# lab-emi/CleanUMamba

Hardware: AMD Instinct MI355X
Metric: audio samples/sec/node (train step, E8, 10s@16kHz) (higher is better)
Workload: dtype f16; 1 GPU; CleanUMamba-E8 (41.4M) full train step: fwd + L1 + multi-res STFT loss + bwd + grad all-reduce + clip + Adam; 10 s @ 16 kHz clips; global_batch=16, batch_per_gpu=16, clip_samples=160000, parallelism=dp1, weights=random init (reference init, seed 0)

## Files before the change

cleanumamba_amd/csrc/gemm_tn.hip:

```cpp
#include "common.h"

namespace cum {

typedef __attribute__((ext_vector_type(8))) __bf16 bf16x8;
typedef __attribute__((ext_vector_type(4))) __bf16 bf16x4;
typedef __attribute__((ext_vector_type(8))) _Float16 f16x8;
typedef __attribute__((ext_vector_type(4))) _Float16 f16x4;
typedef __attribute__((ext_vector_type(4))) float f32x4;

struct TnParams {
  const void *dZ, *X;
  float *slab;
  float *bslab;
  int64_t ldz, ldx;
  int64_t M;
  int N, K;
  int Np, Kp;
  int rows_per_split, nsplit;
#ifdef CUM_AB
  int skip_store;
#endif
};

constexpr int TN_T = 128;

template <typename T>
struct TnCfg;
template <>
struct TnCfg<__bf16> {
  static constexpr int EPC = 8, BMK = 64;
  static __device__ __forceinline__ int swz(int row) { return 2 * ((row & 3) | (((row >> 3) & 1) << 2)); }
};
template <>
struct TnCfg<f16> : TnCfg<__bf16> {};
template <>
struct TnCfg<float> {
  static constexpr int EPC = 4, BMK = 32;
  static __device__ __forceinline__ int swz(int row) { return 4 * (row & 7); }
};

template <typename T>
__global__ __launch_bounds__(256) __attribute__((amdgpu_waves_per_eu(sizeof(T) == 4 ? 2 : 3, 3))) void gemm_tn_kernel(const TnParams p) {
  constexpr int EPC = TnCfg<T>::EPC, BMK = TnCfg<T>::BMK;
  constexpr int CPR = TN_T / EPC;
// ... 579 lines not shown
#undef CUM_MFMA
#undef CUM_HALFQ
#undef CUM_BIAS
#undef CUM_STAGE

  float *slab = p.slab + (int64_t)sp * p.Np * p.Kp;
#pragma unroll
  for (int ni = 0; ni < 4; ++ni) {
    const int n = n0 + wn * 64 + ni * 16 + r;
#pragma unroll
    for (int h = 0; h < 2; ++h)
#pragma unroll
      for (int ki = 0; ki < 4; ++ki) {
        const int k = k0 + wk * 128 + h * 64 + ki * 16 + 4 * g;
        *reinterpret_cast<float4 *>(slab + (int64_t)n * p.Kp + k) =
            make_float4(acc[h][ni][ki][0], acc[h][ni][ki][1], acc[h][ni][ki][2], acc[h][ni][ki][3]);
      }
  }
  if (bias_wave) p.bslab[(int64_t)sp * p.Np + n0 + wn * 64 + 16 * g + r] = bacc[0];
}

#endif

template <typename T>
__global__ __launch_bounds__(512) void gemm_tn9_kernel(const TnParams p) {
  static_assert(sizeof(T) == 2, "16-bit element types only");
  constexpr int UNIT = 64 * 16;
  __shared__ uint4 lds_all[2 * 4 * UNIT];

  const int tid = threadIdx.x, lane = tid & 63;
  const int wave = uniform(tid >> 6);
  const int wk = wave >> 2, wn = wave & 3;
  const int g = lane >> 4, r = lane & 15;
  const int ntn = p.Np / 256, ntk = p.Kp / 256, tiles = ntn * ntk;
  const int w = (int)(blockIdx.x & 7) * (int)(gridDim.x >> 3) + (int)(blockIdx.x >> 3);
  if (w >= tiles * p.nsplit) return;
  const int sp = w / tiles, tile = w % tiles;
  const int n0 = (tile % ntn) * 256, k0 = (tile / ntn) * 256;
  const int64_t m_begin = (int64_t)sp * p.rows_per_split;
  int64_t m_end = m_begin + p.rows_per_split;
  m_end = m_end < p.M ? m_end : p.M;
  const int len = (int)(m_end - m_begin);
  const int nk = (len + 63) / 64;
  const int rem = len - 64 * (nk - 1);
  const T *dZ = static_cast<const T *>(p.dZ);
  const T *X = static_cast<const T *>(p.X);
  const bool bias_wave = p.bslab != nullptr && k0 == 0 && wk == 0;

  typedef __attribute__((address_space(3))) void *lds_ptr;
  typedef const __attribute__((address_space(1))) void *glb_ptr;
  const int64_t stepx = 128 * p.ldx, stepz = 128 * p.ldz;
  const char *xb = reinterpret_cast<const char *>(X + k0) + m_begin * p.ldx * 2;
  const char *zb = reinterpret_cast<const char *>(dZ + n0) + m_begin * p.ldz * 2;
  unsigned xo[2], zo[2];
#pragma unroll
  for (int it = 0; it < 2; ++it) {
    const int pos = it * 512 + tid;
    const int row = pos >> 4;
    const int clog = (pos & 15) ^ TnCfg<T>::swz(row);
    const int rowc = row < rem ? row : rem - 1;
// ... 193 lines not shown
#endif
  float *slab = p.slab + (int64_t)sp * p.Np * p.Kp;
#pragma unroll
  for (int ni = 0; ni < 4; ++ni) {
    const int n = n0 + wn * 64 + ni * 16 + r;
#pragma unroll
    for (int h = 0; h < 2; ++h)
#pragma unroll
      for (int ki = 0; ki < 4; ++ki) {
        const int k = k0 + wk * 128 + h * 64 + ki * 16 + 4 * g;
        *reinterpret_cast<float4 *>(slab + (int64_t)n * p.Kp + k) =
            make_float4(acc[h][ni][ki][0], acc[h][ni][ki][1], acc[h][ni][ki][2], acc[h][ni][ki][3]);
      }
  }
  if (bias_wave) p.bslab[(int64_t)sp * p.Np + n0 + wn * 64 + 16 * g + r] = bacc[0];
}

struct ReduceJob {
  const float *in;
  float *out;
  int64_t in_slab, out_slab, ld_out;
  int ld_in, rows, cols4;
};

__global__ __launch_bounds__(256) void tn_reduce_kernel(const ReduceJob j0, const ReduceJob j1, int nb0, int S) {
  __shared__ float4 red[4][64];
  const bool first = (int)blockIdx.x < nb0;
  const ReduceJob &j = first ? j0 : j1;
  const int bx = first ? blockIdx.x : blockIdx.x - nb0;
  const int v = bx * 64 + (threadIdx.x & 63);
  const int sl = threadIdx.x >> 6;
  const int chunks = gridDim.y, ch = blockIdx.y;
  const int per = (S + chunks - 1) / chunks;
  const int s0 = ch * per;
  int s1 = s0 + per;
  s1 = s1 < S ? s1 : S;
  const int64_t total = (int64_t)j.rows * j.cols4;
  float4 a = make_float4(0.f, 0.f, 0.f, 0.f), b = a;
  int n = 0, k = 0;
  if (v < total) {
    n = v / j.cols4;
    k = (v % j.cols4) * 4;
    const float *base = j.in + (int64_t)n * j.ld_in + k;
    int s = s0 + sl;
    for (; s + 4 < s1; s += 8) {
      const float4 x = *reinterpret_cast<const float4 *>(base + (int64_t)s * j.in_slab);
      const float4 y = *reinterpret_cast<const float4 *>(base + (int64_t)(s + 4) * j.in_slab);
      a.x += x.x; a.y += x.y; a.z += x.z; a.w += x.w;
      b.x += y.x; b.y += y.y; b.z += y.z; b.w += y.w;
    }
    for (; s < s1; s += 4) {
      const float4 x = *reinterpret_cast<const float4 *>(base + (int64_t)s * j.in_slab);
      a.x += x.x; a.y += x.y; a.z += x.z; a.w += x.w;
    }
    a.x += b.x; a.y += b.y; a.z += b.z; a.w += b.w;
// ... 7 lines not shown
      const float4 t = red[q][threadIdx.x];
      r.x += t.x; r.y += t.y; r.z += t.z; r.w += t.w;
    }
    *reinterpret_cast<float4 *>(j.out + (int64_t)ch * j.out_slab + (int64_t)n * j.ld_out + k) = r;
  }
}

}

using namespace cum;

static int tn8_enabled() { return (int)cum_knob("CUM_TN8", 1); }

static bool tn_use8(int64_t M, int32_t N, int32_t K, int32_t dtype) {
  return is16(dtype) && N % 256 == 0 && K % 256 == 0 && M >= 256 && tn8_enabled();
}

static bool tn_use_stream(int64_t M, int32_t N, int32_t K, int32_t dtype) {
  if (!is16(dtype) || tn_use8(M, N, K, dtype) || cum_knob("CUM_TN_STREAM", 1) == 0) return false;
  const int np = (N + TN_T - 1) / TN_T, kp = (K + TN_T - 1) / TN_T;
  return np * kp == 2 && M >= 256 * 64 * 8;
}

static void tn_plan(int64_t M, int32_t N, int32_t K, int32_t dtype, int *Np, int *Kp, int *S, int *rps) {
  const int force = (int)cum_knob("CUM_TN_SPLITS", 0);
  if (tn_use_stream(M, N, K, dtype)) {
    *Np = (N + TN_T - 1) / TN_T * TN_T;
    *Kp = (K + TN_T - 1) / TN_T * TN_T;
    int64_t rows = (M + 255) / 256;
    if (force > 0) rows = (M + force - 1) / force;
    rows = (rows + 63) / 64 * 64;
    *rps = (int)rows;
    *S = (int)((M + rows - 1) / rows);
    return;
  }
  if (tn_use8(M, N, K, dtype)) {
    *Np = N;
    *Kp = K;
    const int tiles = (N / 256) * (K / 256);
    int64_t want = tiles >= 256 ? 1 : 256 / tiles;
    if (force > 0) want = force;
    const int64_t max_s = (M + 255) / 256;
    if (want > max_s) want = max_s;
    int64_t rows = (M + want - 1) / want;
    rows = (rows + 63) / 64 * 64;
    *rps = (int)rows;
    *S = (int)((M + rows - 1) / rows);
    return;
  }
  *Np = (N + TN_T - 1) / TN_T * TN_T;
  *Kp = (K + TN_T - 1) / TN_T * TN_T;
  const int tiles = (*Np / TN_T) * (*Kp / TN_T);
  const int bmk = is16(dtype) ? 32 : 16;
  const int per_xcd = tiles >= 96 ? 1 : 96 / tiles;
  int64_t want = 8 * per_xcd;
  if (force > 0) want = force;
  const int64_t max_s = (M + 8 * bmk - 1) / (8 * bmk);
  if (want > max_s) want = max_s;
  if (want < 1) want = 1;
  int64_t rows = (M + want - 1) / want;
  rows = (rows + bmk - 1) / bmk * bmk;
  *rps = (int)rows;
  *S = (int)((M + rows - 1) / rows);
  if (*S < 1) *S = 1;
}

static int reduce_chunks(int S) { return S >= 64 ? 16 : 1; }

extern "C" int64_t cum_gemm_tn_workspace_elems(int32_t dtype, int64_t M, int32_t N, int32_t K) {
  int Np, Kp, S, rps;
  tn_plan(M, N, K, dtype, &Np, &Kp, &S, &rps);
  const int64_t C = reduce_chunks(S);
  return (int64_t)S * Np * Kp + (int64_t)S * Np + C * (int64_t)N * K + C * (int64_t)Np;
}

extern "C" int cum_gemm_tn_tile(int32_t dtype, int64_t M, int32_t N, int32_t K) {
  return tn_use8(M, N, K, dtype) ? 256 : tn_use_stream(M, N, K, dtype) ? 384 : TN_T;
}

extern "C" int cum_gemm_tn(int32_t dtype, int64_t M, int32_t N, int32_t K, const void *dZ, int64_t ldz, const void *X,
                           int64_t ldx, float *dW, int64_t ldw, float *db, float *workspace, void *stream) {
  CUM_REQUIRE(dtype_ok(dtype), "gemm_tn: dtype must be CUM_F32, CUM_BF16 or CUM_F16");
  CUM_REQUIRE(dZ && X && dW && workspace && M >= 0 && N > 0 && K > 0, "gemm_tn: bad argument");
  const int epc = is16(dtype) ? 8 : 4;
  CUM_REQUIRE(N % epc == 0 && K % epc == 0 && ldz % epc == 0 && ldx % epc == 0 && ldw % 4 == 0,
              "gemm_tn: N, K and strides must keep 16-byte alignment");
  CUM_REQUIRE(((uintptr_t)dZ & 15) == 0 && ((uintptr_t)X & 15) == 0 && ((uintptr_t)dW & 15) == 0,
              "gemm_tn: pointers must be 16-byte aligned");
  hipStream_t st = (hipStream_t)stream;
  const bool want_bias = db != nullptr;
  if (M == 0) {
    (void)hipMemset2DAsync(dW, sizeof(float) * ldw, 0, sizeof(float) * K, N, st);
    if (db) (void)hipMemsetAsync(db, 0, sizeof(float) * N, st);
    return CUM_OK;
  }
  int Np, Kp, S, rps;
  tn_plan(M, N, K, dtype, &Np, &Kp, &S, &rps);
  TnParams p{};
  p.dZ = dZ; p.X = X; p.ldz = ldz; p.ldx = ldx; p.M = M; p.N = N; p.K = K; p.Np = Np; p.Kp = Kp;
  p.rows_per_split = rps;
  p.nsplit = S;
  p.slab = workspace;
  p.bslab = want_bias ? workspace + (int64_t)S * Np * Kp : nullptr;
#ifdef CUM_AB
  p.skip_store = (int)cum_knob("CUM_TN_NOSTORE", 0);
#endif
  dim3 grid(8 * (Np / TN_T) * (Kp / TN_T) * ((S + 7) / 8)), block(256);
  if (tn_use8(M, N, K, dtype)) {
    const int items = (N / 256) * (K / 256) * S;
    const dim3 grid8(8 * ((items + 7) / 8)), block8(512);
#ifdef CUM_AB
    if (cum_knob("CUM_TN9", 1) == 0) {
      if (dtype == CUM_BF16) hipLaunchKernelGGL(gemm_tn8_kernel<__bf16>, grid8, block8, 0, st, p);
      else hipLaunchKernelGGL(gemm_tn8_kernel<f16>, grid8, block8, 0, st, p);
    } else
#endif
    if (dtype == CUM_BF16)
      hipLaunchKernelGGL(gemm_tn9_kernel<__bf16>, grid8, block8, 0, st, p);
    else
      hipLaunchKernelGGL(gemm_tn9_kernel<f16>, grid8, block8, 0, st, p);
  } else if (tn_use_stream(M, N, K, dtype)) {
    CUM_REQUIRE((int64_t)rps * (ldz > ldx ? ldz : ldx) + 512 < (int64_t)1 << 31, "gemm_tn: a row split exceeds 2^31 elements");
    const dim3 gs(S), bs(512);
    if (Np == 128) {
      if (dtype == CUM_BF16) hipLaunchKernelGGL((gemm_tn_stream_kernel<__bf16, 128, 256>), gs, bs, 0, st, p);
      else hipLaunchKernelGGL((gemm_tn_stream_kernel<f16, 128, 256>), gs, bs, 0, st, p);
    } else {
      if (dtype == CUM_BF16) hipLaunchKernelGGL((gemm_tn_stream_kernel<__bf16, 256, 128>), gs, bs, 0, st, p);
      else hipLaunchKernelGGL((gemm_tn_stream_kernel<f16, 256, 128>), gs, bs, 0, st, p);
    }
  } else if (dtype == CUM_BF16)
    hipLaunchKernelGGL(gemm_tn_kernel<__bf16>, grid, block, 0, st, p);
  else if (dtype == CUM_F16)
    hipLaunchKernelGGL(gemm_tn_kernel<f16>, grid, block, 0, st, p);
  else
    hipLaunchKernelGGL(gemm_tn_kernel<float>, grid, block, 0, st, p);
  CUM_CHECK_LAUNCH();
#ifdef CUM_AB
  if (cum_knob("CUM_TN_NOREDUCE", 0)) return CUM_OK;
#endif
  const int C = reduce_chunks(S);
  float *part = workspace + (int64_t)S * Np * Kp + (int64_t)S * Np;
  float *bpart = part + (int64_t)C * N * K;
  const int cols4 = K / 4, bc4 = N / 4;
  const int gx = (int)(((int64_t)N * cols4 + 63) / 64), bx = want_bias ? (bc4 + 63) / 64 : 0;
  if (C == 1) {
    const ReduceJob w{p.slab, dW, (int64_t)Np * Kp, 0, ldw, Kp, N, cols4};
    const ReduceJob bj{p.bslab, db, (int64_t)Np, 0, N, Np, 1, bc4};
    hipLaunchKernelGGL(tn_reduce_kernel, dim3(gx + bx, 1), dim3(256), 0, st, w, bj, gx, S);
  } else {
    const ReduceJob w1{p.slab, part, (int64_t)Np * Kp, (int64_t)N * K, (int64_t)K, Kp, N, cols4};
    const ReduceJob b1{p.bslab, bpart, (int64_t)Np, (int64_t)Np, (int64_t)Np, Np, 1, bc4};
    hipLaunchKernelGGL(tn_reduce_kernel, dim3(gx + bx, C), dim3(256), 0, st, w1, b1, gx, S);
    const ReduceJob w2{part, dW, (int64_t)N * K, 0, ldw, K, N, cols4};
    const ReduceJob b2{bpart, db, (int64_t)Np, 0, N, Np, 1, bc4};
    hipLaunchKernelGGL(tn_reduce_kernel, dim3(gx + bx, 1), dim3(256), 0, st, w2, b2, gx, C);
  }
  CUM_CHECK_LAUNCH();
  return CUM_OK;
}
```

cleanumamba_amd/hip.py:

```python
import ctypes
import os

import torch

_HERE = os.path.dirname(os.path.abspath(__file__))
LIB_PATH = os.environ.get("CUM_LIB") or os.path.join(_HERE, "libcleanumamba_hip.so")

c_i32, c_i64, c_f32p, c_vp = ctypes.c_int32, ctypes.c_int64, ctypes.c_void_p, ctypes.c_void_p


class ScanShape(ctypes.Structure):
    _fields_ = [("batch", c_i32), ("dim", c_i32), ("dstate", c_i32), ("len", c_i32),
                ("u_sb", c_i64), ("u_sd", c_i64), ("u_sl", c_i64),
                ("dt_sb", c_i64), ("dt_sd", c_i64), ("dt_sl", c_i64),
                ("z_sb", c_i64), ("z_sd", c_i64), ("z_sl", c_i64),
                ("o_sb", c_i64), ("o_sd", c_i64), ("o_sl", c_i64),
                ("B_sb", c_i64), ("B_sn", c_i64), ("B_sl", c_i64),
                ("C_sb", c_i64), ("C_sn", c_i64), ("C_sl", c_i64),
                ("delta_softplus", c_i32), ("io_dtype", c_i32)]


class ScanGradStrides(ctypes.Structure):
    _fields_ = [("du_sb", c_i64), ("du_sd", c_i64), ("du_sl", c_i64),
                ("dd_sb", c_i64), ("dd_sd", c_i64), ("dd_sl", c_i64),
# ... 55 lines not shown
    "cum_selective_scan_fwd_from": (c_i32, [ctypes.POINTER(ScanShape)] + [_P] * 13),
    "cum_scan_fwd_keeps_y": (c_i32, [c_i32, c_i32, c_i32, c_i32, c_i32]),
    "cum_scan_bwd_workspace_elems": (c_i64, [c_i32, c_i32, c_i32, c_i32]),
    "cum_selective_scan_bwd": (c_i32, [ctypes.POINTER(ScanShape), ctypes.POINTER(ScanGradStrides)] + [_P] * 21),
    "cum_scan_bwd_tp_workspace_elems": (c_i64, [c_i32, c_i32, c_i32, c_i32]),
    "cum_selective_scan_bwd_tp": (c_i32, [ctypes.POINTER(ScanShape), ctypes.POINTER(ScanGradStrides)] + [_P] * 21),
    "cum_selective_state_update": (c_i32, [c_i32, c_i32, c_i32, _P, _P, _P, _P, _P, c_i64, _P, c_i64,
                                           _P, _P, _P, c_i32, _P, _P]),
    "cum_causal_conv1d_fwd": (c_i32, [ctypes.POINTER(ConvShape)] + [_P] * 5),
    "cum_causal_conv1d_fwd_from": (c_i32, [ctypes.POINTER(ConvShape)] + [_P] * 7),
    "cum_conv_bwd_workspace_elems": (c_i64, [c_i32, c_i32, c_i32, c_i32]),
    "cum_causal_conv1d_bwd": (c_i32, [ctypes.POINTER(ConvShape)] + [_P] * 5 + [c_i64] * 3 + [_P] * 4),
    "cum_causal_conv1d_update": (c_i32, [c_i32, c_i32, c_i32, _P, _P, _P, _P, c_i32, _P, _P]),
    "cum_gemm_nt": (c_i32, [ctypes.POINTER(GemmDesc)] + [_P] * 8),
    "cum_gemm_nt_tile": (c_i32, [ctypes.POINTER(GemmDesc)]),
    "cum_gemm_tn_tile": (c_i32, [c_i32, c_i64, c_i32, c_i32]),
    "cum_glu_bwd_gate": (c_i32, [c_i32, c_i64, c_i32, c_i32, _P, c_i64, _P, c_i64, _P, c_i64, _P, c_i64, _P]),
    "cum_glu_bwd": (c_i32, [c_i32, c_i64, c_i32, c_i32, _P, c_i64, _P, c_i64, _P, _P]),
    "cum_relu_bwd": (c_i32, [c_i32, c_i64, c_i32, _P, c_i64, _P, c_i64, _P, c_i64, c_i64, c_i64, _P]),
    "cum_colsum_workspace_elems": (c_i64, [c_i64, c_i32]),
    "cum_colsum": (c_i32, [c_i32, c_i64, c_i32, _P, c_i64, _P, _P, _P]),
    "cum_gemm_tn_workspace_elems": (c_i64, [c_i32, c_i64, c_i32, c_i32]),
    "cum_gemm_tn": (c_i32, [c_i32, c_i64, c_i32, c_i32, _P, c_i64, _P, c_i64, _P, c_i64, _P, _P, _P]),
    "cum_stft_frames": (c_i32, [_P, c_i64, c_i64, c_i64, c_i32, c_i32, c_i32, _P, _P, c_i64, _P]),
    "cum_stft_loss_workspace_elems": (c_i64, [c_i64, c_i64]),
    "cum_stft_loss_fwd": (c_i32, [_P, _P, c_i64, c_i64, c_i32, c_i64, _P, _P, _P]),
    "cum_stft_loss_bwd": (c_i32, [_P, _P, c_i64, c_i64, c_i32, c_i64, _P, _P, _P, _P, _P]),
    "cum_stft_fold": (c_i32, [_P, c_i64, c_i64, c_i32, c_i32, c_i32, _P, c_i64, _P, c_i64, c_i32, _P]),
    "cum_gather": (c_i32, [c_i32, _P, _P, c_i64, c_i32, _P, _P]),
    "cum_pack2d": (c_i32, [_P, _P, _P, c_i32, _P, c_i32, _P, _P]),
    "cum_add_layernorm_fwd": (c_i32, [c_i32, c_i32, c_i64, c_i32, c_i32, _P, c_i64, c_i64, _P, _P, _P, ctypes.c_float,
                                      _P, _P, _P, _P, _P]),
    "cum_add_layernorm_bwd_workspace_elems": (c_i64, [c_i32]),
    "cum_add_layernorm_bwd": (c_i32, [c_i32, c_i32, c_i64, c_i32] + [_P] * 12),
    "cum_small_linear": (c_i32, [c_i32, c_i32, c_i32, _P, c_i64, _P, _P, _P, c_i64, _P]),
    "cum_mamba_step_supported": (c_i32, [c_i32] * 5),
    "cum_mamba_step": (c_i32, [c_i32] * 6 + [ctypes.c_float] + [_P] * 20),
    "cum_stream_window_update": (c_i32, [c_i32, c_i32, c_i32, c_i32, c_i32, _P, _P, c_i64, c_i64, c_i32, _P, _P, c_i64, _P]),
    "cum_stream_tail_rows": (c_i32, [c_i32, c_i32, c_i32, c_i32, _P, c_i64, c_i32, _P, c_i64, _P]),
    "cum_stream_overlap_add": (c_i32, [c_i32, c_i32, c_i32, c_i32, c_i32, _P, c_i64, _P, _P, _P, c_i64, _P, c_i64, c_i32, _P]),
    "cum_stream_hop_plan_ints": (c_i32, []),
    "cum_stream_hop_max_lds_bytes": (c_i32, []),
    "cum_stream_hop": (c_i32, [_P, _P, _P, c_i64, c_i32, _P, c_i64, _P, c_i64, c_i32, c_i32, _P]),
    "cum_stream_hop_slots": (c_i32, [_P, _P, _P, c_i64, c_i32, _P, _P, c_i32, _P, c_i64, _P, c_i64, c_i32, _P]),
    "cum_stream_pool_stage": (c_i32, [_P, c_i64, c_i32, _P, _P, c_i32, _P, c_i64, _P, c_i64, _P]),
    "cum_fft_plan_create": (c_i32, [c_i32, c_i32, c_i64, ctypes.POINTER(ctypes.c_void_p), ctypes.POINTER(c_i64)]),
# ... 166 lines not shown
```

cleanumamba_amd/network/convstack.py:

```python
import ctypes
import os

import numpy as np
import torch

from .. import hip


def rup(x, m):
    return (x + m - 1) // m * m


class Geo:

    def __init__(self, B, T, C):
        self.B, self.T, self.C = B, T, C
        self.P = T + 2
        self.Cp = rup(C, 8)
        self.M = B * self.P
        self.slack = 2 + (128 + self.Cp - 1) // self.Cp
        self.R = 1 + self.M + self.slack

    def new(self, dtype, device, zero=False):
        if zero:
# ... 33 lines not shown
    d.allow_split_k = 2 if split_k else int(_SPLIT_K_OK)
    if geo is not None:
        d.zero_head, d.zero_tail = geo.head, geo.tail
    P = lambda t, off: None if t is None else ctypes.c_void_p(t.data_ptr() + off * (esz if t.dtype == dt else 0))
    with torch.cuda.device(A.device):
        hip.check(hip.lib().cum_gemm_nt(ctypes.byref(d), P(A, a_off), P(Wp, 0), hip.ptr(bias), P(res, r_off),
                                        P(out, o_off), P(aux, x_off), P(aux2, y_off), hip.stream_ptr()))


_SPLIT_K_OK = False


class small_m_gemms:

    def __enter__(self):
        global _SPLIT_K_OK
        self.prev, _SPLIT_K_OK = _SPLIT_K_OK, True

    def __exit__(self, *exc):
        global _SPLIT_K_OK
        _SPLIT_K_OK = self.prev


def wgrad(dZ, z_off, ldz, N, X, x_off, ldx, K, M, want_bias=True, out=None, out_w=None, out_b=None):
    lib = hip.lib()
    dc = hip.dtype_code(dZ.dtype)
    dev = dZ.device
    if out_w is not None:
        dW = out_w.view(N, K)
        db = (out_b if out_b is not None else torch.empty(N, dtype=torch.float32, device=dev)) if want_bias else None
    elif out is not None:
        arena, off = out
        dW = arena[off:off + N * K].view(N, K)
        db = arena[off + N * K:off + N * K + N] if want_bias else None
    else:
        dW = torch.empty(N, K, dtype=torch.float32, device=dev)
        db = torch.empty(N, dtype=torch.float32, device=dev) if want_bias else None
    ws = torch.empty(max(lib.cum_gemm_tn_workspace_elems(dc, M, N, K), 1), dtype=torch.float32, device=dev)
    esz = dZ.element_size()
    with torch.cuda.device(dev):
        hip.check(lib.cum_gemm_tn(dc, M, N, K, ctypes.c_void_p(dZ.data_ptr() + z_off * esz), ldz,
                                  ctypes.c_void_p(X.data_ptr() + x_off * esz), ldx, hip.ptr(dW), K, hip.ptr(db),
                                  hip.ptr(ws), hip.stream_ptr()))
    return dW, db


def colsum(X, x_off, ld, M, n):
    lib = hip.lib()
    out = torch.empty(n, dtype=torch.float32, device=X.device)
    ws = torch.empty(max(lib.cum_colsum_workspace_elems(M, n), 1), dtype=torch.float32, device=X.device)
    with torch.cuda.device(X.device):
        hip.check(lib.cum_colsum(hip.dtype_code(X.dtype), M, n, ctypes.c_void_p(X.data_ptr() + x_off * X.element_size()),
                                 ld, hip.ptr(out), hip.ptr(ws), hip.stream_ptr()))
    return out


_INDEX_CACHE = {}


def gather(src_flat, idx32, dtype, out=None):
    if out is None or out.numel() != idx32.numel() or out.dtype != dtype or out.device != src_flat.device:
        out = torch.empty(idx32.numel(), dtype=dtype, device=src_flat.device)
    if not src_flat.is_contiguous():
        src_flat = src_flat.contiguous()
    with torch.cuda.device(src_flat.device):
        hip.check(hip.lib().cum_gather(hip.dtype_code(src_flat.dtype), hip.ptr(src_flat), hip.ptr(idx32), idx32.numel(),
                                       hip.dtype_code(dtype), hip.ptr(out), hip.stream_ptr()))
# ... 830 lines not shown
    ybuf = go.new(dt, dev)
    keep = relu and skip is not None
    if keep and _SIGN_MASK:
        act = torch.empty(go.R * go.Cp // 4, dtype=torch.uint8, device=dev)
        gemm(xbuf, 0, gi.Cp, wp, bp, ybuf, go.Cp, N, gi.M, gi.P, gi.T + 1, hip.EPI_RELU, N,
             res=skip, r_off=go.Cp, ldr=N, aux=act[go.Cp // 4:], x_off=0, ldz=N, geo=go, mask_bits=True)
        return ybuf, act
    act = go.new(dt, dev) if keep else None
    gemm(xbuf, 0, gi.Cp, wp, bp, ybuf, go.Cp, N, gi.M, gi.P, gi.T + 1, hip.EPI_RELU if relu else hip.EPI_BIAS, N,
         res=skip, r_off=go.Cp, ldr=N, aux=act, x_off=go.Cp, ldz=N, geo=go)
    return ybuf, (act if keep else (ybuf if relu else None))


def _glu_bwd(z, ybuf, dy, go):
    G = z.shape[1] // 16
    dz = torch.empty(go.M, G * 32, dtype=z.dtype, device=z.device)
    with torch.cuda.device(z.device):
        hip.check(hip.lib().cum_glu_bwd_gate(hip.dtype_code(z.dtype), go.M, G, go.Cp, hip.ptr(z), G * 16,
                                             hip.ptr(ybuf[1:]), go.Cp, hip.ptr(dy[1:]), go.Cp, hip.ptr(dz), G * 32,
                                             hip.stream_ptr()))
    return dz


def _glu_wgrad(dz, xbuf, gi, M, out):
    G32 = dz.shape[1]
    wgrad(dz, 0, G32, G32, xbuf, gi.Cp, gi.Cp, gi.Cp, M, out=out)


def _glu_dgrad_weights(w, gi, G32, dt):
    sh = tuple(w.shape)
    Nd, Kd = rup(gi.Cp, 16), rup(G32, bk_of(dt))
    return take(w, ("glu_dgrad", sh, Nd, Kd),
                lambda: torch.nn.functional.pad(lay_glu_fwd(sh, G32, Nd).t(), (0, Kd - G32)), dt)


_ENC_BITS = os.environ.get("CUM_ENC_BITS", "1") != "0"
_ENC0_FUSED = os.environ.get("CUM_ENC0_FUSED", "1") != "0"


def _enc0_ok(w1, w2, gi, gm, go, dt):
    return (_ENC0_FUSED and dt in hip.HALF_TYPES and tuple(w1.shape) == (64, 1, 4) and tuple(w2.shape) == (128, 64, 1)
            and gi.C == 1 and gi.Cp == 8 and gm.C == 64 and go.C == 64 and w1.dtype == torch.float32)


def _enc0_w2p(w2, gm, dt):
    sh = tuple(w2.shape)
    G = (sh[0] // 2 + 15) // 16
    Kp = rup(gm.Cp, bk_of(dt))
    wp = take(w2, ("glu_fwd", sh, G * 32, Kp), lambda: lay_glu_fwd(sh, G * 32, Kp), dt)
# ... 178 lines not shown
            return out
        key = ("enc", tuple(shapes), tuple((g[0].Cp, g[1].Cp) for g in geos), tuple(z.shape[1] for z in zs))

        def deliver(lo, hi):
            grads[4 * lo:4 * hi] = arena.deliver((key, lo, hi), params[4 * lo:4 * hi], shapes[4 * lo:4 * hi],
                                                 lambda: parts(lo, hi))
        cut = E - 3 if E > 3 else 0
        sink = grad_sink(params) if cut > 0 else None
        early = sink is not None and getattr(sink[0], "early_announce", False)
        for i in reversed(range(E)):
            gi, gm, go = geos[i]
            w1, b1, w2, b2 = params[4 * i:4 * i + 4]
            if dz is None:
                if dys[i] is None:
                    raise RuntimeError("EncoderStack: the deepest output must be used")
                dz = _glu_bwd(zs[i], bufs[i + 1], dys[i].contiguous(), go)
            G32 = dz.shape[1]
            y1 = y1s[i]
            if y1 is None:
                if not ctx.needs_input_grad[0]:
                    _enc0_bwd(dz, bufs[0], w1, b1, w2, gm, go, arena.out(0), arena.out(1))
                    break
                y1 = _conv_relu_fwd(bufs[0], w1, b1, gi, gm)
            _glu_wgrad(dz, y1, gm, go.M, arena.out(2 * i + 1))
            wt = _glu_dgrad_weights(w2, gm, G32, dt)
            dzc = gm.new(dt, dev)
            if bits[i] is not None:
                gemm(dz, 0, G32, wt, None, dzc, gm.Cp, gm.Cp, gm.M, gm.P, gm.T, hip.EPI_MASK, gm.Cp,
                     res=bits[i][gm.Cp // 4:], r_off=0, ldr=gm.Cp, geo=gm, mask_bits=True)
            else:
                gemm(dz, 0, G32, wt, None, dzc, gm.Cp, gm.Cp, gm.M, gm.P, gm.T, hip.EPI_MASK, gm.Cp,
                     res=y1, r_off=gm.Cp, ldr=gm.Cp, geo=gm)
            sh = tuple(w1.shape)
            wgrad(dzc, gm.Cp, gm.Cp, gm.Cp, bufs[i], gi.Cp, 2 * gi.Cp, 4 * gi.Cp, gm.M, out=arena.out(2 * i))
            dz = None
            if early and i == cut:
                deliver(cut, E)
            if i == 0 and not ctx.needs_input_grad[0]:
                break
            Nd, Kd = rup(2 * gi.Cp, 16), rup(2 * gm.Cp, bk_of(dt))
            wd = take(w1, ("conv_dgrad", sh, gi.Cp, gm.Cp, Nd, Kd), lambda: lay_conv_dgrad(sh, gi.Cp, gm.Cp, Nd, Kd), dt)
            ext = None if i == 0 or dys[i - 1] is None else dys[i - 1].contiguous()
            if i > 0 and gi.Cp % 16 == 0:
                dz = torch.empty(gi.M, 2 * gi.Cp, dtype=dt, device=dev)
                gemm(dzc, 0, gm.Cp, wd, None, dz, 0, 4 * gi.Cp, gm.M, gm.P, gm.T + 1, hip.EPI_GLU_BWD, 2 * gi.Cp,
                     res=ext, r_off=gi.Cp, ldr=2 * gi.Cp, aux=zs[i - 1], x_off=0, ldz=2 * gi.Cp,
                     aux2=bufs[i], y_off=gi.Cp, ldy=2 * gi.Cp, gate_only=True)
                continue
            dx = gi.new(dt, dev)
            gemm(dzc, 0, gm.Cp, wd, None, dx, gi.Cp, 2 * gi.Cp, gm.M, gm.P, gm.T + 1, hip.EPI_BIAS, 2 * gi.Cp, geo=gi)
            if i == 0:
                dx0 = dx
            else:
                dz = _glu_bwd(zs[i - 1], bufs[i], dx if ext is None else dx + ext, gi)
        deliver(0, cut if early else E)
        return (dx0, None, None, *grads)

# ... 73 lines not shown

        def parts():
            out = []
            for j in range(E):
                gi, gg, go = geos[j]
                sh1, sht = shapes3[3 * j], shapes3[3 * j + 2]
                G32 = g32s[j]
                out.append(arena.dw_index(2 * j, _invert(lay_glu_fwd(sh1, G32, gi.Cp), sh1)))
                out.append(arena.db_index(2 * j, _invert(lay_glu_vec(sh1[0]), (sh1[0],))))
                out.append(arena.dw_index(2 * j + 1, _invert(lay_convt_fwd(sht, gg.Cp, go.Cp, 2 * go.Cp, 2 * gg.Cp), sht)))
            return out
        key = ("dec", tuple(shapes3), tuple((g[0].Cp, g[1].Cp, g[2].Cp) for g in geos), tuple(g32s))
        for j in reversed(range(E)):
            gi, gg, go = geos[j]
            w1, b1, wt, bt = params[4 * j:4 * j + 4]
            sht = tuple(wt.shape)
            if j == E - 1 and ctx.fused_last:
                (ab, ao), nk = arena.out(2 * j + 1), 2 * go.Cp * 2 * gg.Cp
                du, dpre = _dec7_bwd(dpre, us[j], acts[j - 1][gi.Cp // 4:], w1, b1, wt, gi, arena.out(2 * j), (ab, ao))
                grads[4 * j + 3] = _convt_bias_grad(bt, ab[ao + nk:ao + nk + 2 * go.Cp], go.Cp, sht[1], wt.dtype)
                if j - 1 < ctx.n_skips:
                    dskips[j - 1] = du
                continue
            _, dbp = wgrad(dpre, go.Cp, 2 * go.Cp, 2 * go.Cp, gs[j], 0, gg.Cp, 2 * gg.Cp, gg.M, out=arena.out(2 * j + 1))
            grads[4 * j + 3] = _convt_bias_grad(bt, dbp, go.Cp, sht[1], wt.dtype)
            Nd, Kd = rup(gg.Cp, 16), rup(4 * go.Cp, bk_of(dt))
            wc = take(wt, ("convt_dgrad", sht, go.Cp, Nd, Kd), lambda: lay_convt_dgrad(sht, go.Cp, Nd, Kd), dt)
            z = zs[j]
            G32 = 2 * z.shape[1]
            if gg.Cp % 16 == 0:
                dz = torch.empty(gg.M, G32, dtype=dt, device=dev)
                gemm(dpre, go.Cp, 2 * go.Cp, wc, None, dz, 0, G32, gg.M, gg.P, gg.T, hip.EPI_GLU_BWD, gg.Cp,
                     aux=z, x_off=0, ldz=gg.Cp, aux2=gs[j], y_off=gg.Cp, ldy=gg.Cp, gate_only=True)
            else:
                dg = gg.new(dt, dev)
                gemm(dpre, go.Cp, 2 * go.Cp, wc, None, dg, gg.Cp, gg.Cp, gg.M, gg.P, gg.T, hip.EPI_BIAS, gg.Cp, geo=gg)
                dz = _glu_bwd(z, gs[j], dg, gg)
            _glu_wgrad(dz, us[j], gi, gg.M, arena.out(2 * j))
            w1t = _glu_dgrad_weights(w1, gi, G32, dt)
            du = gi.new(dt, dev)
            if j > 0 and acts[j - 1] is not None:
                dpre = gi.new(dt, dev)
                bits = acts[j - 1].dtype == torch.uint8
                gemm(dz, 0, G32, w1t, None, dpre, gi.Cp, gi.Cp, gi.M, gi.P, gi.T, hip.EPI_MASK, gi.Cp,
                     res=acts[j - 1][gi.Cp // 4:] if bits else acts[j - 1], r_off=0 if bits else gi.Cp, ldr=gi.Cp,
                     aux=du, x_off=gi.Cp, ldz=gi.Cp, geo=gi, mask_bits=bits)
            else:
                gemm(dz, 0, G32, w1t, None, du, gi.Cp, gi.Cp, gi.M, gi.P, gi.T, hip.EPI_BIAS, gi.Cp, geo=gi)
                dpre = du
            if j > 0 and j - 1 < ctx.n_skips:
                dskips[j - 1] = du
        three = [params[4 * j + k] for j in range(E) for k in range(3)]
        un = arena.deliver(key, three, shapes3, parts)
        for j in range(E):
            grads[4 * j:4 * j + 3] = un[3 * j:3 * j + 3]
        return (du, None, None, None, *dskips, *grads)
```

include/cleanumamba_hip.h:

```cpp
#ifndef CLEANUMAMBA_HIP_H
#define CLEANUMAMBA_HIP_H

#include <stdint.h>

#ifdef __cplusplus
extern "C" {
#endif

#define CUM_OK 0
#define CUM_EINVAL (-1)
#define CUM_ELAUNCH (-2)
#define CUM_EWORKSPACE (-3)

#define CUM_ABI_VERSION 16

int cum_abi_version(void);
const char *cum_last_error(void);

int cum_scan_chunk(void);

#define CUM_SCAN_SOFTPLUS 1
#define CUM_SCAN_A_IS_LOG 2
typedef struct {
  int32_t batch, dim, dstate, len;
// ... 104 lines not shown
int cum_gemm_nt(const cum_gemm_desc *d, const void *A, const void *W, const float *bias,
                const void *res, void *out, void *aux, const void *aux2, void *stream);
int cum_gemm_nt_tile(const cum_gemm_desc *d);

int cum_glu_bwd(int32_t dtype, int64_t M, int32_t n_groups, int32_t n_out, const void *Z,
                int64_t ldz, const void *dOut, int64_t ldo, void *dZ, void *stream);
int cum_glu_bwd_gate(int32_t dtype, int64_t M, int32_t n_groups, int32_t n_out, const void *Bg,
                     int64_t ldb, const void *Y, int64_t ldy, const void *dOut, int64_t ldo, void *dZ,
                     int64_t ldz, void *stream);

int cum_relu_bwd(int32_t dtype, int64_t M, int32_t n_cols, const void *Y, int64_t ldy,
                 const void *dOut, int64_t ldo, void *dZ, int64_t ldz, int64_t zero_head,
                 int64_t zero_tail, void *stream);

int64_t cum_colsum_workspace_elems(int64_t M, int32_t n_cols);
int cum_colsum(int32_t dtype, int64_t M, int32_t n_cols, const void *X, int64_t ld, float *out,
               float *workspace, void *stream);

int64_t cum_gemm_tn_workspace_elems(int32_t dtype, int64_t M, int32_t N, int32_t K);
int cum_gemm_tn(int32_t dtype, int64_t M, int32_t N, int32_t K, const void *dZ, int64_t ldz,
                const void *X, int64_t ldx, float *dW, int64_t ldw, float *db, float *workspace,
                void *stream);
int cum_gemm_tn_tile(int32_t dtype, int64_t M, int32_t N, int32_t K);

int cum_stft_frames(const float *x, int64_t batch, int64_t len, int64_t x_stride_b, int32_t n_fft, int32_t hop,
                    int32_t win_length, const float *window, float *frames, int64_t n_frames, void *stream);
int64_t cum_stft_loss_workspace_elems(int64_t batch, int64_t n_frames);
int cum_stft_loss_fwd(const float *spec_x, const float *spec_y, int64_t batch, int64_t n_frames, int32_t bins,
                      int64_t frame0, float *workspace, float *stats, void *stream);
int cum_stft_loss_bwd(const float *spec_x, const float *spec_y, int64_t batch, int64_t n_frames, int32_t bins,
                      int64_t frame0, const float *stats, const float *g_sc, const float *g_mag, float *zspec,
                      void *stream);
int cum_stft_fold(const float *dframes, int64_t batch, int64_t len, int32_t n_fft, int32_t hop, int32_t win_length,
                  const float *window, int64_t n_frames, float *dx, int64_t dx_stride_b, int32_t accumulate,
                  void *stream);

int cum_gather(int32_t src_dtype, const void *src, const int32_t *idx, int64_t n, int32_t dst_dtype, void *dst,
               void *stream);

int cum_pack2d(const float *src, const void *jobs, const int32_t *tiles, int32_t n_tiles, const int32_t *tables,
               int32_t dst_dtype, void *dst, void *stream);

int cum_fft_plan_create(int32_t kind, int32_t n, int64_t batch, void **plan, int64_t *work_bytes);
int cum_fft_plan_destroy(void *plan);
int cum_fft_exec(void *plan, float *in, float *out, int32_t inverse, void *work, void *stream);

// ... 188 lines not shown
```

Measured before the change: 136.5 million audio samples/s.

## Batch paired conv weight-gradient GEMMs into one grouped launch with shared reduce

Adds a paired TN weight-gradient GEMM that runs two same-M problems in a single grouped kernel launch, with the block range split between them. The split-K reduction kernel now handles up to four jobs, so both problems reduce together. The encoder and decoder backward passes hold the first wgrad and launch it alongside the second. The aim is fewer launches and better CU occupancy for small-tile wgrads, at the cost of a larger combined workspace and deferred gradient availability.

```diff
diff --git a/cleanumamba_amd/csrc/gemm_tn.hip b/cleanumamba_amd/csrc/gemm_tn.hip
--- a/cleanumamba_amd/csrc/gemm_tn.hip
+++ b/cleanumamba_amd/csrc/gemm_tn.hip
@@ -20,6 +20,11 @@
 #ifdef CUM_AB
   int skip_store;
 #endif
+};
+
+struct TnPair {
+  TnParams a, b;
+  int blocks_a;
 };
 
 constexpr int TN_T = 128;
@@ -645,8 +650,27 @@
 
 #endif
 
-template <typename T>
-__global__ __launch_bounds__(512) void gemm_tn9_kernel(const TnParams p) {
+__device__ __forceinline__ void tn9_decode(const TnParams &p, int lb, int nb, int &sp, int &tile, bool &live) {
+  const int tiles = (p.Np / 256) * (p.Kp / 256);
+  const int w = (lb & 7) * (nb >> 3) + (lb >> 3);
+  live = w < tiles * p.nsplit;
+  sp = w / tiles;
+  tile = w % tiles;
+}
+__device__ __forceinline__ const TnParams &tn9_item(const TnParams &p, int &sp, int &tile, bool &live) {
+  tn9_decode(p, (int)blockIdx.x, (int)gridDim.x, sp, tile, live);
+  return p;
+}
+__device__ __forceinline__ const TnParams &tn9_item(const TnPair &pp, int &sp, int &tile, bool &live) {
+  const int bid = (int)blockIdx.x;
+  const bool second = bid >= pp.blocks_a;
+  const TnParams &p = second ? pp.b : pp.a;
+  tn9_decode(p, second ? bid - pp.blocks_a : bid, second ? (int)gridDim.x - pp.blocks_a : pp.blocks_a, sp, tile, live);
+  return p;
+}
+
+template <typename T, typename P>
+__global__ __launch_bounds__(512) void gemm_tn9_kernel(const P args) {
   static_assert(sizeof(T) == 2, "16-bit element types only");
   constexpr int UNIT = 64 * 16;
   __shared__ uint4 lds_all[2 * 4 * UNIT];
@@ -655,10 +679,11 @@
   const int wave = uniform(tid >> 6);
   const int wk = wave >> 2, wn = wave & 3;
   const int g = lane >> 4, r = lane & 15;
-  const int ntn = p.Np / 256, ntk = p.Kp / 256, tiles = ntn * ntk;
-  const int w = (int)(blockIdx.x & 7) * (int)(gridDim.x >> 3) + (int)(blockIdx.x >> 3);
-  if (w >= tiles * p.nsplit) return;
-  const int sp = w / tiles, tile = w % tiles;
+  int sp, tile;
+  bool live;
+  const TnParams &p = tn9_item(args, sp, tile, live);
+  if (!live) return;
+  const int ntn = p.Np / 256;
   const int n0 = (tile % ntn) * 256, k0 = (tile / ntn) * 256;
   const int64_t m_begin = (int64_t)sp * p.rows_per_split;
   int64_t m_end = m_begin + p.rows_per_split;
@@ -898,15 +923,28 @@
   int64_t in_slab, out_slab, ld_out;
   int ld_in, rows, cols4;
 };
-
-__global__ __launch_bounds__(256) void tn_reduce_kernel(const ReduceJob j0, const ReduceJob j1, int nb0, int S) {
+struct ReduceJobs {
+  ReduceJob j[4];
+  int end[4], S[4], chunks[4];
+};
+
+__global__ __launch_bounds__(256) void tn_reduce_kernel(const ReduceJobs t) {
   __shared__ float4 red[4][64];
-  const bool first = (int)blockIdx.x < nb0;
-  const ReduceJob &j = first ? j0 : j1;
-  const int bx = first ? blockIdx.x : blockIdx.x - nb0;
+  int ji = 0, first = 0;
+#pragma unroll
+  for (int i = 0; i < 3; ++i)
+    if ((int)blockIdx.x >= t.end[i]) {
+      ji = i + 1;
+      first = t.end[i];
+    }
+  const ReduceJob &j = ji == 0 ? t.j[0] : ji == 1 ? t.j[1] : ji == 2 ? t.j[2] : t.j[3];
+  const int bx = (int)blockIdx.x - first;
   const int v = bx * 64 + (threadIdx.x & 63);
   const int sl = threadIdx.x >> 6;
-  const int chunks = gridDim.y, ch = blockIdx.y;
+  const int S = ji == 0 ? t.S[0] : ji == 1 ? t.S[1] : ji == 2 ? t.S[2] : t.S[3];
+  const int chunks = ji == 0 ? t.chunks[0] : ji == 1 ? t.chunks[1] : ji == 2 ? t.chunks[2] : t.chunks[3];
+  const int ch = blockIdx.y;
+  if (ch >= chunks) return;
   const int per = (S + chunks - 1) / chunks;
   const int s0 = ch * per;
   int s1 = s0 + per;
@@ -960,6 +998,22 @@
   return np * kp == 2 && M >= 256 * 64 * 8;
 }
 
+static void tn8_split(int64_t M, int tiles, int *S, int *rps) {
+  const int force = (int)cum_knob("CUM_TN_SPLITS", 0);
+  int64_t want = tiles >= 256 ? 1 : 256 / tiles;
+  if (force > 0) want = force;
+  const int64_t max_s = (M + 255) / 256;
+  if (want > max_s) want = max_s;
+  int64_t rows = (M + want - 1) / want;
+  rows = (rows + 63) / 64 * 64;
+  *rps = (int)rows;
+  *S = (int)((M + rows - 1) / rows);
+}
+
+static bool tn_pair_ok(int32_t dtype, int64_t M, int32_t N0, int32_t K0, int32_t N1, int32_t K1) {
+  return tn_use8(M, N0, K0, dtype) && tn_use8(M, N1, K1, dtype);
+}
+
 static void tn_plan(int64_t M, int32_t N, int32_t K, int32_t dtype, int *Np, int *Kp, int *S, int *rps) {
   const int force = (int)cum_knob("CUM_TN_SPLITS", 0);
   if (tn_use_stream(M, N, K, dtype)) {
@@ -975,15 +1029,7 @@
   if (tn_use8(M, N, K, dtype)) {
     *Np = N;
     *Kp = K;
-    const int tiles = (N / 256) * (K / 256);
-    int64_t want = tiles >= 256 ? 1 : 256 / tiles;
-    if (force > 0) want = force;
-    const int64_t max_s = (M + 255) / 256;
-    if (want > max_s) want = max_s;
-    int64_t rows = (M + want - 1) / want;
-    rows = (rows + 63) / 64 * 64;
-    *rps = (int)rows;
-    *S = (int)((M + rows - 1) / rows);
+    tn8_split(M, (N / 256) * (K / 256), S, rps);
     return;
   }
   *Np = (N + TN_T - 1) / TN_T * TN_T;
@@ -1005,19 +1051,8 @@
 
 static int reduce_chunks(int S) { return S >= 64 ? 16 : 1; }
 
-extern "C" int64_t cum_gemm_tn_workspace_elems(int32_t dtype, int64_t M, int32_t N, int32_t K) {
-  int Np, Kp, S, rps;
-  tn_plan(M, N, K, dtype, &Np, &Kp, &S, &rps);
-  const int64_t C = reduce_chunks(S);
-  return (int64_t)S * Np * Kp + (int64_t)S * Np + C * (int64_t)N * K + C * (int64_t)Np;
-}
-
-extern "C" int cum_gemm_tn_tile(int32_t dtype, int64_t M, int32_t N, int32_t K) {
-  return tn_use8(M, N, K, dtype) ? 256 : tn_use_stream(M, N, K, dtype) ? 384 : TN_T;
-}
-
-extern "C" int cum_gemm_tn(int32_t dtype, int64_t M, int32_t N, int32_t K, const void *dZ, int64_t ldz, const void *X,
-                           int64_t ldx, float *dW, int64_t ldw, float *db, float *workspace, void *stream) {
+static int tn_check(int32_t dtype, int64_t M, int32_t N, int32_t K, const void *dZ, int64_t ldz, const void *X, int64_t ldx,
+                    const float *dW, int64_t ldw, const float *workspace) {
   CUM_REQUIRE(dtype_ok(dtype), "gemm_tn: dtype must be CUM_F32, CUM_BF16 or CUM_F16");
   CUM_REQUIRE(dZ && X && dW && workspace && M >= 0 && N > 0 && K > 0, "gemm_tn: bad argument");
   const int epc = is16(dtype) ? 8 : 4;
@@ -1025,6 +1060,73 @@
               "gemm_tn: N, K and strides must keep 16-byte alignment");
   CUM_REQUIRE(((uintptr_t)dZ & 15) == 0 && ((uintptr_t)X & 15) == 0 && ((uintptr_t)dW & 15) == 0,
               "gemm_tn: pointers must be 16-byte aligned");
+  return CUM_OK;
+}
+
+struct TnReduceProblem {
+  const float *slab, *bslab;
+  float *dW;
+  int64_t ldw;
+  float *db;
+  int N, K, Np, Kp, S;
+  float *part, *bpart;
+};
+
+static void tn_reduce(const TnReduceProblem *r, int n, hipStream_t st) {
+  ReduceJobs t1{}, t2{};
+  int end1 = 0, end2 = 0, cmax = 1;
+  for (int i = 0; i < 2; ++i) {
+    if (i < n) {
+      const TnReduceProblem &q = r[i];
+      const int C = reduce_chunks(q.S);
+      const int cols4 = q.K / 4, bc4 = q.N / 4;
+      const int64_t nk = (int64_t)q.N * q.K;
+      const int gw = (int)((nk / 4 + 63) / 64), gb = q.bslab ? (bc4 + 63) / 64 : 0;
+      cmax = C > cmax ? C : cmax;
+      t1.S[2 * i] = t1.S[2 * i + 1] = q.S;
+      t1.chunks[2 * i] = t1.chunks[2 * i + 1] = C;
+      if (C == 1) {
+        t1.j[2 * i] = ReduceJob{q.slab, q.dW, (int64_t)q.Np * q.Kp, 0, q.ldw, q.Kp, q.N, cols4};
+        t1.j[2 * i + 1] = ReduceJob{q.bslab, q.db, (int64_t)q.Np, 0, q.N, q.Np, 1, bc4};
+      } else {
+        t1.j[2 * i] = ReduceJob{q.slab, q.part, (int64_t)q.Np * q.Kp, nk, (int64_t)q.K, q.Kp, q.N, cols4};
+        t1.j[2 * i + 1] = ReduceJob{q.bslab, q.bpart, (int64_t)q.Np, (int64_t)q.Np, (int64_t)q.Np, q.Np, 1, bc4};
+        t2.j[2 * i] = ReduceJob{q.part, q.dW, nk, 0, q.ldw, q.K, q.N, cols4};
+        t2.j[2 * i + 1] = ReduceJob{q.bpart, q.db, (int64_t)q.Np, 0, q.N, q.Np, 1, bc4};
+        t2.S[2 * i] = t2.S[2 * i + 1] = C;
+        t2.chunks[2 * i] = t2.chunks[2 * i + 1] = 1;
+        end2 += gw;
+        t2.end[2 * i] = end2;
+        end2 += gb;
+        t2.end[2 * i + 1] = end2;
+      }
+      end1 += gw;
+      t1.end[2 * i] = end1;
+      end1 += gb;
+      t1.end[2 * i + 1] = end1;
+    } else {
+      t1.end[2 * i] = t1.end[2 * i + 1] = end1;
+    }
+    if (i >= n || reduce_chunks(r[i].S) == 1) t2.end[2 * i] = t2.end[2 * i + 1] = end2;
+  }
+  hipLaunchKernelGGL(tn_reduce_kernel, dim3(end1, cmax), dim3(256), 0, st, t1);
+  if (end2 > 0) hipLaunchKernelGGL(tn_reduce_kernel, dim3(end2, 1), dim3(256), 0, st, t2);
+}
+
+extern "C" int64_t cum_gemm_tn_workspace_elems(int32_t dtype, int64_t M, int32_t N, int32_t K) {
+  int Np, Kp, S, rps;
+  tn_plan(M, N, K, dtype, &Np, &Kp, &S, &rps);
+  const int64_t C = reduce_chunks(S);
+  return (int64_t)S * Np * Kp + (int64_t)S * Np + C * (int64_t)N * K + C * (int64_t)Np;
+}
+
+extern "C" int cum_gemm_tn_tile(int32_t dtype, int64_t M, int32_t N, int32_t K) {
+  return tn_use8(M, N, K, dtype) ? 256 : tn_use_stream(M, N, K, dtype) ? 384 : TN_T;
+}
+
+extern "C" int cum_gemm_tn(int32_t dtype, int64_t M, int32_t N, int32_t K, const void *dZ, int64_t ldz, const void *X,
+                           int64_t ldx, float *dW, int64_t ldw, float *db, float *workspace, void *stream) {
+  if (int rc = tn_check(dtype, M, N, K, dZ, ldz, X, ldx, dW, ldw, workspace)) return rc;
   hipStream_t st = (hipStream_t)stream;
   const bool want_bias = db != nullptr;
   if (M == 0) {
@@ -1054,9 +1156,9 @@
     } else
 #endif
     if (dtype == CUM_BF16)
-      hipLaunchKernelGGL(gemm_tn9_kernel<__bf16>, grid8, block8, 0, st, p);
+      hipLaunchKernelGGL((gemm_tn9_kernel<__bf16, TnParams>), grid8, block8, 0, st, p);
     else
-      hipLaunchKernelGGL(gemm_tn9_kernel<f16>, grid8, block8, 0, st, p);
+      hipLaunchKernelGGL((gemm_tn9_kernel<f16, TnParams>), grid8, block8, 0, st, p);
   } else if (tn_use_stream(M, N, K, dtype)) {
     CUM_REQUIRE((int64_t)rps * (ldz > ldx ? ldz : ldx) + 512 < (int64_t)1 << 31, "gemm_tn: a row split exceeds 2^31 elements");
     const dim3 gs(S), bs(512);
@@ -1077,23 +1179,63 @@
 #ifdef CUM_AB
   if (cum_knob("CUM_TN_NOREDUCE", 0)) return CUM_OK;
 #endif
-  const int C = reduce_chunks(S);
+  TnReduceProblem r{p.slab, p.bslab, dW, ldw, db, N, K, Np, Kp, S};
   float *part = workspace + (int64_t)S * Np * Kp + (int64_t)S * Np;
-  float *bpart = part + (int64_t)C * N * K;
-  const int cols4 = K / 4, bc4 = N / 4;
-  const int gx = (int)(((int64_t)N * cols4 + 63) / 64), bx = want_bias ? (bc4 + 63) / 64 : 0;
-  if (C == 1) {
-    const ReduceJob w{p.slab, dW, (int64_t)Np * Kp, 0, ldw, Kp, N, cols4};
-    const ReduceJob bj{p.bslab, db, (int64_t)Np, 0, N, Np, 1, bc4};
-    hipLaunchKernelGGL(tn_reduce_kernel, dim3(gx + bx, 1), dim3(256), 0, st, w, bj, gx, S);
-  } else {
-    const ReduceJob w1{p.slab, part, (int64_t)Np * Kp, (int64_t)N * K, (int64_t)K, Kp, N, cols4};
-    const ReduceJob b1{p.bslab, bpart, (int64_t)Np, (int64_t)Np, (int64_t)Np, Np, 1, bc4};
-    hipLaunchKernelGGL(tn_reduce_kernel, dim3(gx + bx, C), dim3(256), 0, st, w1, b1, gx, S);
-    const ReduceJob w2{part, dW, (int64_t)N * K, 0, ldw, K, N, cols4};
-    const ReduceJob b2{bpart, db, (int64_t)Np, 0, N, Np, 1, bc4};
-    hipLaunchKernelGGL(tn_reduce_kernel, dim3(gx + bx, 1), dim3(256), 0, st, w2, b2, gx, C);
-  }
+  r.part = part;
+  r.bpart = part + (int64_t)reduce_chunks(S) * N * K;
+  tn_reduce(&r, 1, st);
   CUM_CHECK_LAUNCH();
   return CUM_OK;
 }
+
+extern "C" int64_t cum_gemm_tn_pair_workspace_elems(int32_t dtype, int64_t M, int32_t N0, int32_t K0, int32_t N1,
+                                                    int32_t K1) {
+  if (!tn_pair_ok(dtype, M, N0, K0, N1, K1)) {
+    const int64_t a = cum_gemm_tn_workspace_elems(dtype, M, N0, K0), b = cum_gemm_tn_workspace_elems(dtype, M, N1, K1);
+    return a > b ? a : b;
+  }
+  return cum_gemm_tn_workspace_elems(dtype, M, N0, K0) + cum_gemm_tn_workspace_elems(dtype, M, N1, K1);
+}
+
+extern "C" int cum_gemm_tn_pair(int32_t dtype, int64_t M0, int32_t N0, int32_t K0, const void *dZ0, int64_t ldz0,
+                                const void *X0, int64_t ldx0, float *dW0, int64_t ldw0, float *db0, int64_t M1, int32_t N1,
+                                int32_t K1, const void *dZ1, int64_t ldz1, const void *X1, int64_t ldx1, float *dW1,
+                                int64_t ldw1, float *db1, float *workspace, void *stream) {
+  CUM_REQUIRE(M0 == M1, "gemm_tn_pair: the two problems must have the same M");
+  if (int rc = tn_check(dtype, M0, N0, K0, dZ0, ldz0, X0, ldx0, dW0, ldw0, workspace)) return rc;
+  if (int rc = tn_check(dtype, M1, N1, K1, dZ1, ldz1, X1, ldx1, dW1, ldw1, workspace)) return rc;
+  const int64_t M = M0;
+  if (!tn_pair_ok(dtype, M, N0, K0, N1, K1)) {
+    if (int rc = cum_gemm_tn(dtype, M, N0, K0, dZ0, ldz0, X0, ldx0, dW0, ldw0, db0, workspace, stream)) return rc;
+    return cum_gemm_tn(dtype, M, N1, K1, dZ1, ldz1, X1, ldx1, dW1, ldw1, db1, workspace, stream);
+  }
+  hipStream_t st = (hipStream_t)stream;
+  const int t0 = (N0 / 256) * (K0 / 256), t1 = (N1 / 256) * (K1 / 256);
+  int S0, rps0, S1, rps1;
+  tn8_split(M, t0, &S0, &rps0);
+  tn8_split(M, t1, &S1, &rps1);
+  const int64_t C0 = reduce_chunks(S0), C1 = reduce_chunks(S1), nk0 = (int64_t)N0 * K0, nk1 = (int64_t)N1 * K1;
+  float *slab0 = workspace, *slab1 = slab0 + S0 * nk0, *bslab0 = slab1 + S1 * nk1, *bslab1 = bslab0 + (int64_t)S0 * N0;
+  float *part0 = bslab1 + (int64_t)S1 * N1, *part1 = part0 + C0 * nk0, *bpart0 = part1 + C1 * nk1, *bpart1 = bpart0 + C0 * N0;
+  TnPair pp{};
+  pp.a.dZ = dZ0; pp.a.X = X0; pp.a.ldz = ldz0; pp.a.ldx = ldx0; pp.a.M = M; pp.a.N = N0; pp.a.K = K0; pp.a.Np = N0; pp.a.Kp = K0;
+  pp.b.dZ = dZ1; pp.b.X = X1; pp.b.ldz = ldz1; pp.b.ldx = ldx1; pp.b.M = M; pp.b.N = N1; pp.b.K = K1; pp.b.Np = N1; pp.b.Kp = K1;
+  pp.a.rows_per_split = rps0; pp.a.nsplit = S0;
+  pp.b.rows_per_split = rps1; pp.b.nsplit = S1;
+  pp.a.slab = slab0;
+  pp.b.slab = slab1;
+  pp.a.bslab = db0 ? bslab0 : nullptr;
+  pp.b.bslab = db1 ? bslab1 : nullptr;
+  pp.blocks_a = 8 * ((t0 * S0 + 7) / 8);
+  const dim3 grid(pp.blocks_a + 8 * ((t1 * S1 + 7) / 8)), block(512);
+  if (dtype == CUM_BF16)
+    hipLaunchKernelGGL((gemm_tn9_kernel<__bf16, TnPair>), grid, block, 0, st, pp);
+  else
+    hipLaunchKernelGGL((gemm_tn9_kernel<f16, TnPair>), grid, block, 0, st, pp);
+  CUM_CHECK_LAUNCH();
+  const TnReduceProblem r[2] = {{slab0, pp.a.bslab, dW0, ldw0, db0, N0, K0, N0, K0, S0, part0, bpart0},
+                                {slab1, pp.b.bslab, dW1, ldw1, db1, N1, K1, N1, K1, S1, part1, bpart1}};
+  tn_reduce(r, 2, st);
+  CUM_CHECK_LAUNCH();
+  return CUM_OK;
+}
diff --git a/cleanumamba_amd/hip.py b/cleanumamba_amd/hip.py
--- a/cleanumamba_amd/hip.py
+++ b/cleanumamba_amd/hip.py
@@ -101,6 +101,8 @@
     "cum_colsum": (c_i32, [c_i32, c_i64, c_i32, _P, c_i64, _P, _P, _P]),
     "cum_gemm_tn_workspace_elems": (c_i64, [c_i32, c_i64, c_i32, c_i32]),
     "cum_gemm_tn": (c_i32, [c_i32, c_i64, c_i32, c_i32, _P, c_i64, _P, c_i64, _P, c_i64, _P, _P, _P]),
+    "cum_gemm_tn_pair_workspace_elems": (c_i64, [c_i32, c_i64, c_i32, c_i32, c_i32, c_i32]),
+    "cum_gemm_tn_pair": (c_i32, [c_i32] + [c_i64, c_i32, c_i32, _P, c_i64, _P, c_i64, _P, c_i64, _P] * 2 + [_P, _P]),
     "cum_stft_frames": (c_i32, [_P, c_i64, c_i64, c_i64, c_i32, c_i32, c_i32, _P, _P, c_i64, _P]),
     "cum_stft_loss_workspace_elems": (c_i64, [c_i64, c_i64]),
     "cum_stft_loss_fwd": (c_i32, [_P, _P, c_i64, c_i64, c_i32, c_i64, _P, _P, _P]),
diff --git a/cleanumamba_amd/network/convstack.py b/cleanumamba_amd/network/convstack.py
--- a/cleanumamba_amd/network/convstack.py
+++ b/cleanumamba_amd/network/convstack.py
@@ -79,7 +79,23 @@
         _SPLIT_K_OK = self.prev
 
 
-def wgrad(dZ, z_off, ldz, N, X, x_off, ldx, K, M, want_bias=True, out=None, out_w=None, out_b=None):
+_WGRAD_PAIR = True
+
+
+class _HeldWgrad:
+
+    def __init__(self, dZ, z_off, ldz, N, X, x_off, ldx, K, M, dW, db):
+        self.dZ, self.z_off, self.ldz, self.N, self.X, self.x_off, self.ldx, self.K, self.M = dZ, z_off, ldz, N, X, x_off, ldx, K, M
+        self.dW, self.db = dW, db
+        self.launched = False
+
+    def args(self):
+        esz = self.dZ.element_size()
+        return (self.M, self.N, self.K, ctypes.c_void_p(self.dZ.data_ptr() + self.z_off * esz), self.ldz,
+                ctypes.c_void_p(self.X.data_ptr() + self.x_off * esz), self.ldx, hip.ptr(self.dW), self.K, hip.ptr(self.db))
+
+
+def wgrad(dZ, z_off, ldz, N, X, x_off, ldx, K, M, want_bias=True, out=None, out_w=None, out_b=None, hold=False, pair=None):
     lib = hip.lib()
     dc = hip.dtype_code(dZ.dtype)
     dev = dZ.device
@@ -93,13 +109,35 @@
     else:
         dW = torch.empty(N, K, dtype=torch.float32, device=dev)
         db = torch.empty(N, dtype=torch.float32, device=dev) if want_bias else None
+    if hold and _WGRAD_PAIR:
+        return _HeldWgrad(dZ, z_off, ldz, N, X, x_off, ldx, K, M, dW, db)
+    if pair is not None and not pair.launched:
+        wgrad_pair(pair, _HeldWgrad(dZ, z_off, ldz, N, X, x_off, ldx, K, M, dW, db))
+        return dW, db
     ws = torch.empty(max(lib.cum_gemm_tn_workspace_elems(dc, M, N, K), 1), dtype=torch.float32, device=dev)
     esz = dZ.element_size()
     with torch.cuda.device(dev):
         hip.check(lib.cum_gemm_tn(dc, M, N, K, ctypes.c_void_p(dZ.data_ptr() + z_off * esz), ldz,
                                   ctypes.c_void_p(X.data_ptr() + x_off * esz), ldx, hip.ptr(dW), K, hip.ptr(db),
                                   hip.ptr(ws), hip.stream_ptr()))
+    if hold:
+        h = _HeldWgrad(dZ, z_off, ldz, N, X, x_off, ldx, K, M, dW, db)
+        h.launched = True
+        return h
     return dW, db
+
+
+def wgrad_pair(a, b):
+    if a.M != b.M or a.dZ.dtype != b.dZ.dtype or a.X.dtype != a.dZ.dtype or b.X.dtype != a.dZ.dtype:
+        raise RuntimeError("wgrad_pair: the two problems must share M and the element type")
+    lib = hip.lib()
+    dc = hip.dtype_code(a.dZ.dtype)
+    dev = a.dZ.device
+    ws = torch.empty(max(lib.cum_gemm_tn_pair_workspace_elems(dc, a.M, a.N, a.K, b.N, b.K), 1), dtype=torch.float32,
+                     device=dev)
+    with torch.cuda.device(dev):
+        hip.check(lib.cum_gemm_tn_pair(dc, *a.args(), *b.args(), hip.ptr(ws), hip.stream_ptr()))
+    a.launched = b.launched = True
 
 
 def colsum(X, x_off, ld, M, n):
@@ -976,9 +1014,9 @@
     return dz
 
 
-def _glu_wgrad(dz, xbuf, gi, M, out):
+def _glu_wgrad(dz, xbuf, gi, M, out, hold=False, pair=None):
     G32 = dz.shape[1]
-    wgrad(dz, 0, G32, G32, xbuf, gi.Cp, gi.Cp, gi.Cp, M, out=out)
+    return wgrad(dz, 0, G32, G32, xbuf, gi.Cp, gi.Cp, gi.Cp, M, out=out, hold=hold, pair=pair)
 
 
 def _glu_dgrad_weights(w, gi, G32, dt):
@@ -1203,7 +1241,7 @@
                     _enc0_bwd(dz, bufs[0], w1, b1, w2, gm, go, arena.out(0), arena.out(1))
                     break
                 y1 = _conv_relu_fwd(bufs[0], w1, b1, gi, gm)
-            _glu_wgrad(dz, y1, gm, go.M, arena.out(2 * i + 1))
+            held = _glu_wgrad(dz, y1, gm, go.M, arena.out(2 * i + 1), hold=True)
             wt = _glu_dgrad_weights(w2, gm, G32, dt)
             dzc = gm.new(dt, dev)
             if bits[i] is not None:
@@ -1213,7 +1251,7 @@
                 gemm(dz, 0, G32, wt, None, dzc, gm.Cp, gm.Cp, gm.M, gm.P, gm.T, hip.EPI_MASK, gm.Cp,
                      res=y1, r_off=gm.Cp, ldr=gm.Cp, geo=gm)
             sh = tuple(w1.shape)
-            wgrad(dzc, gm.Cp, gm.Cp, gm.Cp, bufs[i], gi.Cp, 2 * gi.Cp, 4 * gi.Cp, gm.M, out=arena.out(2 * i))
+            wgrad(dzc, gm.Cp, gm.Cp, gm.Cp, bufs[i], gi.Cp, 2 * gi.Cp, 4 * gi.Cp, gm.M, out=arena.out(2 * i), pair=held)
             dz = None
             if early and i == cut:
                 deliver(cut, E)
@@ -1333,8 +1371,8 @@
                 if j - 1 < ctx.n_skips:
                     dskips[j - 1] = du
                 continue
-            _, dbp = wgrad(dpre, go.Cp, 2 * go.Cp, 2 * go.Cp, gs[j], 0, gg.Cp, 2 * gg.Cp, gg.M, out=arena.out(2 * j + 1))
-            grads[4 * j + 3] = _convt_bias_grad(bt, dbp, go.Cp, sht[1], wt.dtype)
+            held = wgrad(dpre, go.Cp, 2 * go.Cp, 2 * go.Cp, gs[j], 0, gg.Cp, 2 * gg.Cp, gg.M, out=arena.out(2 * j + 1),
+                         hold=True)
             Nd, Kd = rup(gg.Cp, 16), rup(4 * go.Cp, bk_of(dt))
             wc = take(wt, ("convt_dgrad", sht, go.Cp, Nd, Kd), lambda: lay_convt_dgrad(sht, go.Cp, Nd, Kd), dt)
             z = zs[j]
@@ -1347,7 +1385,8 @@
                 dg = gg.new(dt, dev)
                 gemm(dpre, go.Cp, 2 * go.Cp, wc, None, dg, gg.Cp, gg.Cp, gg.M, gg.P, gg.T, hip.EPI_BIAS, gg.Cp, geo=gg)
                 dz = _glu_bwd(z, gs[j], dg, gg)
-            _glu_wgrad(dz, us[j], gi, gg.M, arena.out(2 * j))
+            _glu_wgrad(dz, us[j], gi, gg.M, arena.out(2 * j), pair=held)
+            grads[4 * j + 3] = _convt_bias_grad(bt, held.db, go.Cp, sht[1], wt.dtype)
             w1t = _glu_dgrad_weights(w1, gi, G32, dt)
             du = gi.new(dt, dev)
             if j > 0 and acts[j - 1] is not None:
diff --git a/include/cleanumamba_hip.h b/include/cleanumamba_hip.h
--- a/include/cleanumamba_hip.h
+++ b/include/cleanumamba_hip.h
@@ -150,6 +150,11 @@
                 const void *X, int64_t ldx, float *dW, int64_t ldw, float *db, float *workspace,
                 void *stream);
 int cum_gemm_tn_tile(int32_t dtype, int64_t M, int32_t N, int32_t K);
+int64_t cum_gemm_tn_pair_workspace_elems(int32_t dtype, int64_t M, int32_t N0, int32_t K0, int32_t N1, int32_t K1);
+int cum_gemm_tn_pair(int32_t dtype, int64_t M0, int32_t N0, int32_t K0, const void *dZ0, int64_t ldz0,
+                     const void *X0, int64_t ldx0, float *dW0, int64_t ldw0, float *db0, int64_t M1,
+                     int32_t N1, int32_t K1, const void *dZ1, int64_t ldz1, const void *X1, int64_t ldx1,
+                     float *dW1, int64_t ldw1, float *db1, float *workspace, void *stream);
 
 int cum_stft_frames(const float *x, int64_t batch, int64_t len, int64_t x_stride_b, int32_t n_fft, int32_t hop,
                     int32_t win_length, const float *window, float *frames, int64_t n_frames, void *stream);
```

Result: no change. 136.5 million audio samples/s, median of 2 (+0.0%).
